# schatty/oprl

Hardware: AMD Instinct MI355X
Metric: learner gradient steps/sec, DDPG batch=256 walker-walk (higher is better)
Workload: dtype f32 (exact-fp32 MFMA)

## Files before the change

### oprl_amd/csrc/batch_rows.h

```cpp
#pragma once
#include "kernels.h"
#include "philox.h"
#include "replay_index.h"

namespace oprl {

constexpr int kMaxEnds = 2048;

__device__ __forceinline__ void load_batch(const BatchSrc& P, int row0, int B, int S, int A,
                                           float* xa, float* xb, float* rS, float* dS, int* meta,
                                           int* endsS) {
  const int tid = threadIdx.x;
  if (P.gather) {
    lds_zero(xa, 2 * kR * kX0Ld);
    const EndsLds ET = stage_ends(P.ends, P.n_eps, endsS, kMaxEnds, tid, kThreads);
    __syncthreads();
    if (tid < kR) {
      const int i = row0 + tid;
      int e = 0, t = 0;
      if (i < B) {
        const u32x4 rnd = philox4x32_10(
            u32x4{(uint32_t)P.counter, (uint32_t)(P.counter >> 32), (uint32_t)i, 0x5a17u},
            (uint32_t)P.seed, (uint32_t)(P.seed >> 32));
        const long ind = (long)bounded_u32(rnd.x, (uint32_t)P.n_transitions);
        long start = 0;
        e = find_episode(P.ends, P.n_eps, ET, ind, &start);
        t = (int)(ind - start);
      }
      meta[tid] = e;
      meta[kR + tid] = t;
    }
    __syncthreads();
    for (int idx = tid; idx < kR * (2 * S + A + 2); idx += kThreads) {
      const int W = 2 * S + A + 2;
      const int row = idx / W, c = idx - row * W;
      if (row0 + row >= B) continue;
      const long e = meta[row], t = meta[kR + row];
      const float* src = P.states + (e * (P.L + 1) + t) * S + c;
      float* dst = xa + row * kX0Ld + c;
      if (c >= S) dst = xb + row * kX0Ld + (c - S);
      if (c >= 2 * S) { src = P.actions + (e * P.L + t) * A + (c - 2 * S); dst = xa + row * kX0Ld + S + (c - 2 * S); }
      if (c == 2 * S + A) { src = P.rewards + e * P.L + t; dst = rS + row; }
      if (c == 2 * S + A + 1) { src = P.dones + e * P.L + t; dst = dS + row; }
      *dst = *src;
    }
  } else {
    constexpr int kPer = (2 * kR * kX0Ld + kThreads - 1) / kThreads;
    float v[kPer];
#pragma unroll
    for (int j = 0; j < kPer; ++j) {
      const int idx = min(tid + j * kThreads, 2 * kR * kX0Ld - 1);
      const int t = idx / (kR * kX0Ld), rem = idx - t * (kR * kX0Ld);
      const int row = rem / kX0Ld, col = rem - row * kX0Ld, gr = row0 + row;
      const bool is_s = gr < B && col < S, is_a = gr < B && t == 0 && col >= S && col < S + A;
      const float* src = P.s;
      if (is_s) src = (t == 0 ? P.s : P.s2) + (size_t)gr * S + col;
      if (is_a) src = P.a + (size_t)gr * A + (col - S);
      const float x = *src;
      v[j] = (is_s || is_a) ? x : 0.f;
    }
#pragma unroll
    for (int j = 0; j < kPer; ++j) {
      const int idx = tid + j * kThreads;
      if (idx < 2 * kR * kX0Ld) xa[idx] = v[j];
    }
    if (tid < kR) {
      const int gr = row0 + tid;
      rS[tid] = gr < B ? P.r[gr] : 0.f;
      dS[tid] = gr < B ? P.d[gr] : 0.f;
    }
  }
}

template <bool WT = false>
__device__ __forceinline__ void prefetch_rows_src(const BatchSrc& N, int S, int Ad, int B, int slice, float* smem);
__device__ __forceinline__ void prefetch_rows_body(const PrefetchJob& J, int slice, float* smem) {
  prefetch_rows_src(J.next, J.S, J.A, J.B, slice, smem);
}
template <bool WT>
__device__ __forceinline__ void prefetch_rows_src(const BatchSrc& N, int S, int Ad, int B, int slice, float* smem) {
  const int tid = threadIdx.x, row0 = slice * kR;
  float* xa = smem;
  float* xb = xa + kR * kX0Ld;
  float* rS = xb + kR * kX0Ld;
  float* dS = rS + kR;
  int* meta = reinterpret_cast<int*>(dS + 2 * kR);
  int* endsS = reinterpret_cast<int*>(rS + 96);
  load_batch(N, row0, B, S, Ad, xa, xb, rS, dS, meta, endsS);
  __syncthreads();
  if constexpr (WT) {
    store_rows_wt(xa, kX0Ld, const_cast<float*>(N.s), S, S, row0, B);
    store_rows_wt(xb, kX0Ld, const_cast<float*>(N.s2), S, S, row0, B);
    store_rows_wt(xa + S, kX0Ld, const_cast<float*>(N.a), Ad, Ad, row0, B);
    if (tid < kR && row0 + tid < B) {
      __hip_atomic_store(const_cast<float*>(N.r) + row0 + tid, rS[tid], __ATOMIC_RELAXED, __HIP_MEMORY_SCOPE_AGENT);
      __hip_atomic_store(const_cast<float*>(N.d) + row0 + tid, dS[tid], __ATOMIC_RELAXED, __HIP_MEMORY_SCOPE_AGENT);
    }
    return;
  }
  store_rows(xa, kX0Ld, const_cast<float*>(N.s), S, S, row0, B);
  store_rows(xb, kX0Ld, const_cast<float*>(N.s2), S, S, row0, B);
  for (int idx = tid; idx < kR * Ad; idx += kThreads) {
    const int row = idx / Ad, col = idx - row * Ad, gr = row0 + row;
    if (gr < B) const_cast<float*>(N.a)[(size_t)gr * Ad + col] = xa[row * kX0Ld + S + col];
  }
  if (tid < kR && row0 + tid < B) {
    const_cast<float*>(N.r)[row0 + tid] = rS[tid];
    const_cast<float*>(N.d)[row0 + tid] = dS[tid];
  }
}

__device__ __forceinline__ void prefetch_rows_direct(const PrefetchJob& J, int slice, int* lds_i, int nt) {
  const int tid = threadIdx.x, row0 = slice * kR, S = J.S, Ad = J.A, B = J.B;
  const BatchSrc& P = J.next;
  int* endsS = lds_i;
  int* meta = lds_i + kMaxEnds;
  const EndsLds ET = stage_ends(P.ends, P.n_eps, endsS, kMaxEnds, tid, nt);
  __syncthreads();
  if (tid < kR) {
    const int i = row0 + tid;
    int e = 0, t = 0;
    if (i < B) {
// ... 28 lines not shown
```

### oprl_amd/csrc/dw_tile_x2.h

```cpp
#pragma once
#include "dw_body.h"

namespace oprl {

constexpr int kDwX2TileK = 64;

__device__ __forceinline__ float wave_max(float v) {
  v = fmaxf(v, __builtin_bit_cast(float, __builtin_amdgcn_update_dpp(0, __builtin_bit_cast(int, v), 0xB1, 0xF, 0xF, true)));
  v = fmaxf(v, __builtin_bit_cast(float, __builtin_amdgcn_update_dpp(0, __builtin_bit_cast(int, v), 0x4E, 0xF, 0xF, true)));
  v = fmaxf(v, __builtin_bit_cast(float, __builtin_amdgcn_update_dpp(0, __builtin_bit_cast(int, v), 0x141, 0xF, 0xF, true)));
  v = fmaxf(v, __builtin_bit_cast(float, __builtin_amdgcn_update_dpp(0, __builtin_bit_cast(int, v), 0x140, 0xF, 0xF, true)));
  const int b = __builtin_bit_cast(int, v);
  const float r0 = __builtin_bit_cast(float, __builtin_amdgcn_readlane(b, 0)), r1 = __builtin_bit_cast(float, __builtin_amdgcn_readlane(b, 16));
  const float r2 = __builtin_bit_cast(float, __builtin_amdgcn_readlane(b, 32)), r3 = __builtin_bit_cast(float, __builtin_amdgcn_readlane(b, 48));
  return fmaxf(fmaxf(r0, r1), fmaxf(r2, r3));
}

__device__ __forceinline__ float ld_ag(const float* p) { return __hip_atomic_load(p, __ATOMIC_RELAXED, __HIP_MEMORY_SCOPE_AGENT); }
__device__ __forceinline__ void st_ag(float* p, float v) { __hip_atomic_store(p, v, __ATOMIC_RELAXED, __HIP_MEMORY_SCOPE_AGENT); }
template <class V16>
__device__ __forceinline__ void st16_wt(float* base, size_t off, const V16 v) {
  static_assert(sizeof(V16) == 16, "16-byte vector");
  st16_agent_at(base, (unsigned)off, __builtin_bit_cast(f32x4, v));
}
// ... 388 lines not shown
      unsigned long long x = 0, xb = 0;
      bool ok = false;
      for (int spin = 0; spin < (1 << 20) && !ok; ++spin) {
        x = __hip_atomic_load(src + tid, __ATOMIC_RELAXED, __HIP_MEMORY_SCOPE_SYSTEM);
        xb = tid < kDwTileN ? __hip_atomic_load(src + 1024 + tid, __ATOMIC_RELAXED, __HIP_MEMORY_SCOPE_SYSTEM) : x;
        ok = (unsigned)(x >> 32) == tag && (unsigned)(xb >> 32) == tag;
        if (!ok) __builtin_amdgcn_s_sleep(2);
      }
      *v = __uint_as_float((unsigned)x);
      *vb = __uint_as_float((unsigned)xb);
      return ok;
    };
    float gs = 0.f, gbs = 0.f;
    bool all_ok = true;
    if (X.rank == owner) {
      for (int r = 0; r < X.world; ++r) {
        float v = gsum, vb = gbw;
        if (r != X.rank) all_ok = get(slot(X.window, r), &v, &vb) && all_ok;
        gs += v;
        gbs += vb;
      }
      if (!all_ok) { gs = __builtin_nanf(""); gbs = gs; }
      for (int p = 0; p < X.world; ++p)
        if (p != X.rank) put(slot(X.peer[p], X.world), gs, gbs);
    } else {
      put(slot(X.peer[owner], X.rank), gsum, gbw);
      all_ok = get(slot(X.window, X.world), &gs, &gbs);
    }
    if (!all_ok) {
      report_expired(X.err, (KERN_DW_XCHG << 8) | SITE_DW_TILE);
      gs = __builtin_nanf(""); gbs = gs;
    }
    gsum = gs;
    gb_x = gbs;
  }
  gsum *= ad.grad_scale;
  if (!ad.do_adam) {
    if (e_ok && I.w_g != nullptr) I.w_g[eo] = gsum;
    if (b_own && I.b_g != nullptr) {
      float gb = 0.f;
#pragma unroll
      for (int q = 0; q < 32; ++q) gb += bpart[q * 16 + tid];
      I.b_g[n_base + tid] = gb * ad.grad_scale;
    }
    return;
  }
  float th_new = 0.f, tt_new = 0.f;
  if (e_ok) {
    float mm = p_m, vv = p_v, th = p_th;
    adam_elem(gsum, mm, vv, th, ad, step_size, bc2_sqrt);
    th_new = th;
    if (polyak) tt_new = polyak_elem(p_tt, th, ad);
    e_m = mm; e_v = vv;
    if (!flagged) {
      st_ag(I.w_m + eo, mm);
      st_ag(I.w_v + eo, vv);
      st_ag(I.w + eo, th);
      if (polyak) st_ag(I.w_t + eo, tt_new);
    }
    if (chained && gate == 2 && kind == 0) st_ag(ov.chain->w3buf[(ov.u + 1) & 1] + eo, th);
  }
  tileW[nl * LDT + kl] = th_new;
  tileT[nl * LDT + kl] = tt_new;
  if (b_own) {
    const int n = n_base + tid;
    float gb = 0.f;
#pragma unroll
    for (int q = 0; q < 32; ++q) gb += bpart[q * 16 + tid];
    if (xchg_on) gb = gb_x;
    gb *= ad.grad_scale;
    float mm = q_m, vv = q_v, th = q_th;
    adam_elem(gb, mm, vv, th, ad, step_size, bc2_sqrt);
    if (I.b16 != nullptr) st_ag(I.b16 + n, th);
    st_ag(I.b_m + n, mm);
    st_ag(I.b_v + n, vv);
    st_ag(I.b + n, th);
    if (b_pol) {
      const float tb = polyak_elem(q_tt, th, ad);
      st_ag(I.b_t + n, tb);
      if (I.bt16 != nullptr) st_ag(I.bt16 + n, tb);
    }
  }
  __syncthreads();

  if constexpr (!P::kX2) {
    if (I.pf != nullptr) {
      const int NSk = cdiv(I.K, 16), NSn = cdiv(I.N, 16);
      const int grp3 = tid >> 8, q = tid & 255, j = q >> 6, l = q & 63, li = l & 15, lk = l >> 4;
      if (grp3 < 2) {
        float* dst = grp3 == 0 ? I.pf : (polyak ? I.tpf : nullptr);
        if (dst != nullptr && 4 * tk + j < NSk && !(flagged && grp3 == 1))
          st16_wt(dst, (((size_t)ptile * NSk + 4 * tk + j) * 64 + l) * 4, ld4((grp3 == 0 ? tileW : tileT) + li * LDT + 16 * j + 4 * lk));
      } else if (grp3 == 2 && I.pb != nullptr) {
        const int ktile = 4 * tk + j;
        if (16 * ktile < I.K) {
          f32x4 w4;
#pragma unroll
          for (int t = 0; t < 4; ++t) w4[t] = tileW[(4 * lk + t) * LDT + 16 * j + li];
          st16_wt(I.pb, (((size_t)ktile * NSn + ptile) * 64 + l) * 4, w4);
        }
      }
    }
  }
  if (!P::kX2 && I.pf16 != nullptr && !I.x2) {
    const int NSk2 = cdiv(I.K, 32), NSn2 = cdiv(I.N, 32);
    typedef __bf16 bf16x4 __attribute__((ext_vector_type(4)));
    if (tid < 256) {
      const int which = tid >> 7, hb = (tid >> 6) & 1, l = tid & 63, li = l & 15, lk = l >> 4;
      float* dst = which == 0 ? I.pf16 : (polyak ? I.tpf16 : nullptr);
      if (dst != nullptr && 2 * tk + hb < NSk2) {
        const float* src = (which == 0 ? tileW : tileT) + li * LDT + 32 * hb;
        st16_wt(dst, (((size_t)ptile * NSk2 + 2 * tk + hb) * 64 + l) * 4, cvt_bf16x8(ld4(src + 4 * lk), ld4(src + 16 + 4 * lk)));
      }
    } else if (tid < 512 && I.pb16 != nullptr) {
      const int q = tid - 256, blk = q >> 6, l = q & 63, li = l & 15, lk = l >> 4;
      const int ktile = 4 * tk + blk;
      if (16 * ktile < I.K) {
        f32x4 w4;
#pragma unroll
        for (int t = 0; t < 4; ++t) w4[t] = tileW[(4 * lk + t) * LDT + 16 * blk + li];
        st8_wt(I.pb16 + (((size_t)ktile * NSn2 + (n_base >> 5)) * 64 + l) * 4 + 2 * ((n_base >> 4) & 1), __builtin_convertvector(w4, bf16x4));
      }
    }
  }
  if (P::kX2 && I.pf16 != nullptr) {
    const int NSk2 = cdiv(I.K, 32), NSn2 = cdiv(I.N, 32);
    typedef _Float16 f16x4 __attribute__((ext_vector_type(4)));
    if (tid < 256) {
      const int which = tid >> 7, hb = (tid >> 6) & 1, l = tid & 63, li = l & 15, lk = l >> 4;
      float* dst = which == 0 ? I.pf16 : (polyak ? I.tpf16 : nullptr);
      if (dst != nullptr && 2 * tk + hb < NSk2 && !(flagged && which == 1)) {
        const float* src = (which == 0 ? tileW : tileT) + li * LDT + 32 * hb;
        f16x8 hi, lo;
        x2_split8(ld4(src + 4 * lk) * PrecX2::kWScale, ld4(src + 16 + 4 * lk) * PrecX2::kWScale, hi, lo);
        const size_t d = ((size_t)ptile * NSk2 + 2 * tk + hb) * 512 + (size_t)l * 4;
        st16_wt(dst, d, hi);
        st16_wt(dst, d + 256, lo);
      }
    } else if (tid < 512 && I.pb16 != nullptr) {
      const int q = tid - 256, blk = q >> 6, l = q & 63, li = l & 15, lk = l >> 4;
      const int ktile = 4 * tk + blk;
      if (16 * ktile < I.K) {
        f32x4 w4;
#pragma unroll
        for (int t = 0; t < 4; ++t) w4[t] = tileW[(4 * lk + t) * LDT + 16 * blk + li];
        const f32x4 vs = w4 * PrecX2::kWScale;
        const f16x4 hi = __builtin_convertvector(vs, f16x4);
        const f32x4 r = vs - __builtin_convertvector(hi, f32x4);
        float* d = I.pb16 + ((size_t)ktile * NSn2 + (n_base >> 5)) * 512 + (size_t)l * 4 + 2 * ((n_base >> 4) & 1);
        st8_wt(d, hi);
        st8_wt(d + 256, __builtin_convertvector(r, f16x4));
      }
    }
  }
  if (flagged) {
    asm volatile("s_waitcnt vmcnt(0)" ::: "memory");
    __syncthreads();
    if (tid == 0)
      __hip_atomic_store(G.done + bx_, (unsigned long long)gtag << 32, __ATOMIC_RELAXED, __HIP_MEMORY_SCOPE_AGENT);
    if (e_ok) {
      st_ag(I.w_m + eo, e_m);
      st_ag(I.w_v + eo, e_v);
      st_ag(I.w + eo, th_new);
      if (polyak) st_ag(I.w_t + eo, tt_new);
    }
    if constexpr (!P::kX2) {
      if (I.pf != nullptr && polyak && I.tpf != nullptr && tid >= 256 && tid < 512) {
        const int NSk = cdiv(I.K, 16);
        const int q = tid & 255, j = q >> 6, l = q & 63, li = l & 15, lk = l >> 4;
        if (4 * tk + j < NSk)
          st16_wt(I.tpf, (((size_t)ptile * NSk + 4 * tk + j) * 64 + l) * 4, ld4(tileT + li * LDT + 16 * j + 4 * lk));
      }
    }
    if (P::kX2 && I.pf16 != nullptr && polyak && I.tpf16 != nullptr && tid >= 128 && tid < 256) {
      const int NSk2 = cdiv(I.K, 32);
      const int hb = (tid >> 6) & 1, l = tid & 63, li = l & 15, lk = l >> 4;
      if (2 * tk + hb < NSk2) {
        const float* src = tileT + li * LDT + 32 * hb;
        f16x8 hi, lo;
        x2_split8(ld4(src + 4 * lk) * PrecX2::kWScale, ld4(src + 16 + 4 * lk) * PrecX2::kWScale, hi, lo);
        const size_t d = ((size_t)ptile * NSk2 + 2 * tk + hb) * 512 + (size_t)l * 4;
        st16_wt(I.tpf16, d, hi);
        st16_wt(I.tpf16, d + 256, lo);
      }
    }
  }
  stamp();
  if (chained) {
    asm volatile("s_waitcnt vmcnt(0)" ::: "memory");
    __syncthreads();
    if (tid == 0)
      __hip_atomic_store((gate == 1 ? ov.chain->ct_fin : ov.chain->at_fin) + bx_, (unsigned long long)gtag << 32, __ATOMIC_RELAXED, __HIP_MEMORY_SCOPE_AGENT);
  }
  }
};

template <class KArgs = DwKArgs, class P = PrecX2>
__device__ __forceinline__ void dw_tile_x2(const KArgs& A, float* lds, int bx, int gate, const DwX2Ovr& ov = DwX2Ovr()) {
  DwX2Tile<KArgs, P> T;
  T.ov = ov;
  T.begin(A, lds, bx, gate);
  T.finish();
}

}
```

### oprl_amd/csrc/fused_ddpg.hip

```cpp
#include <cstddef>
#include <mutex>
#include <type_traits>
#include "kernels.h"
#include "philox.h"
#include "replay_index.h"
#include "batch_rows.h"
#include "slice_head.h"
#include "tp4.h"
#include "dw_body.h"
#include "dw_tile_x2.h"

namespace oprl { constexpr bool kDwTileX2 = true; constexpr bool kMergedTile64 = true; }

namespace oprl {


__device__ __forceinline__ bool cluster_on_one_xcd(const DdpgArgs& A) {
  const int xcc = __builtin_amdgcn_s_getreg((3 << 11) | 20) & 15;
  return A.xcd_local != 0 && ((int)gridDim.x & 7) == 0 && xcc == ((int)blockIdx.x & 7);
}
__global__ void k_xcc_probe(int* out) {
  if (threadIdx.x == 0) out[blockIdx.y * gridDim.x + blockIdx.x] = __builtin_amdgcn_s_getreg((3 << 11) | 20) & 15;
}

// ... 843 lines not shown
template <int WIDTH, bool LEAN, bool SAC, class P = PrecF32, bool WIDE = false>
__global__ __launch_bounds__(kThreads) void k_ddpg_phase2(const DdpgArgs A) { ddpg_phase2_body<WIDTH, LEAN, SAC, P, WIDE>(A); }

template <int WIDTH, bool LEAN, bool SAC, class P = PrecF32>
__global__ __launch_bounds__(kThreads) void k_ddpg_phase2_group(const DdpgArgs* __restrict__ batch) {
  const int S = (int)gridDim.x, R = (int)gridDim.y, n = (int)gridDim.z;
  int l = (int)blockIdx.z, slice = (int)blockIdx.x, by = (int)blockIdx.y;
  if ((n & 7) == 0) {
    const int q = (int)blockIdx.x + S * ((int)blockIdx.y + R * (int)blockIdx.z);
    const int p = q >> 3, inner = p % (S * R);
    l = (q & 7) + 8 * (p / (S * R));
    if constexpr (LEAN) {
      if (inner < 4 * S) { slice = inner >> 2; by = inner & 3; }
      else { slice = inner - 4 * S; by = 4; }
    } else {
      slice = inner % S;
      by = inner / S;
      const int G = batch[0].group_span;
      if (G > 1 && G < 8 && S % G == 0) {
        const int Sp = S / G, pr = p % (Sp * R);
        const int v = (q & 7) + 8 * (p / (Sp * R));
        l = v / G;
        slice = (v - l * G) * Sp + pr % Sp;
        by = pr / Sp;
      } else if (G >= 8) {
        l = (int)blockIdx.z; slice = (int)blockIdx.x; by = (int)blockIdx.y;
      }
    }
  }
  ddpg_phase2_body<WIDTH, LEAN, SAC, P>(batch[l], slice, by);
}


__device__ __forceinline__ void wait_flags(const unsigned long long* flags, int n, unsigned tag, unsigned* err, unsigned code) {
  const int k = (int)threadIdx.x;
  if (k < n) {
    bool ok = false;
    for (int spin = 0; spin < kTpSpin && !ok; ++spin) {
      ok = (unsigned)(__hip_atomic_load(flags + k, __ATOMIC_RELAXED, __HIP_MEMORY_SCOPE_AGENT) >> 32) == tag;
      if (!ok) __builtin_amdgcn_s_sleep(2);
    }
    if (!ok) report_expired(err, code);
  }
}

struct PassCtx {
  unsigned epoch;
  unsigned tag;
  const float* w3;
  const float* cb[3];
  long long* trace;
  const float* pb1_32 = nullptr;
};
template <class P, class KA = DwKArgs, bool PF = true, bool GE = false>
__device__ __forceinline__ int ddpg_phase2m_body(const DdpgArgs& A, const KA* D, int by_in, const PassCtx& cx) {
  static_assert((P::kX2 || GE) && kDwTileX2, "the merged phase 2: PrecX2 learners; with the unit-seed rows (k_ddpg_chain) every arithmetic");
  extern __shared__ __attribute__((aligned(16))) float smem[];
  using LY = FusedLds<256>;
  constexpr int HB = kR * kWL4;
  constexpr int NMC = 8;
  const int B = A.B, S = A.S, Ad = A.A, tid = threadIdx.x;
  const int slice = blockIdx.x, row0 = slice * kR;
  const int y = by_in < 0 ? (int)blockIdx.y : by_in;
  const int yP = NMC, yT = yP + ((PF && A.prefetch_next) ? 1 : 0);
  if (y >= yT) {
    const int tile = (y - yT) * (int)gridDim.x + slice;
    if (tile >= dw_total(*D)) return -1;
    if (A.whole) {
      wait_flags(A.w_flags, 4 * (int)gridDim.x, cx.epoch, A.err, (KERN_PHASE2 << 8) | SITE_DW_GATE);
      __syncthreads();
    }
    return tile;
  }
  float* xa = smem + LY::xa;
  if (PF && y == yP) {
    float* xb = smem + LY::xb;
    float* rS = smem + LY::misc;
    float* dS = rS + kR;
    int* meta = reinterpret_cast<int*>(dS + 2 * kR);
    int* endsS = reinterpret_cast<int*>(smem + LY::misc + 96);
    load_batch(A.next, row0, B, S, Ad, xa, xb, rS, dS, meta, endsS);
    __syncthreads();
    store_rows(xa, kX0Ld, const_cast<float*>(A.next.s), S, S, row0, B);
    store_rows(xb, kX0Ld, const_cast<float*>(A.next.s2), S, S, row0, B);
    for (int idx = tid; idx < kR * Ad; idx += kThreads) {
      const int row = idx / Ad, col = idx - row * Ad, gr = row0 + row;
      if (gr < B) const_cast<float*>(A.next.a)[(size_t)gr * Ad + col] = xa[row * kX0Ld + S + col];
    }
    if (tid < kR && row0 + tid < B) {
      const_cast<float*>(A.next.r)[row0 + tid] = rS[tid];
      const_cast<float*>(A.next.d)[row0 + tid] = dS[tid];
    }
    return -1;
  }
  float* h1 = smem + LY::h;
  float* h2 = h1 + HB;
  float* g2 = h2 + HB;
  float* Wl = g2 + HB;
  float* outS = smem + LY::out;
  float* auxS = smem + LY::aux;
  float* duS = smem + LY::aux2;
  float* scr = smem + LY::scr;
  float* w3s = smem + LY::misc + 96;
  static_assert(2 * HB >= 2 * 8 * 512, "the shard fits the two spare hidden buffers");
  static_assert(kMaxEnds >= kDuLd * 256, "W3 fits the ends table's area");
  Tp tp{y, NMC, A.xbuf + (size_t)slice * kTpStages * A.xnc * kTpBlk, cx.tag, 0,
// ... 28 lines not shown
  const float* wsrc = ((P::kBf16 && cx.pb1_32 != nullptr) ? cx.pb1_32 : A.actor.pb[1]) + (size_t)c * 2 * 16 * 256;
  f32x4 wv[2];
#pragma unroll
  for (int q = 0; q < 2; ++q) wv[q] = ld4c(wsrc + ((size_t)q * kThreads + tid) * 4);
  const int hr = tid >> 6, hc = (tid & 63) * 4;
  f32x4 hv = f32x4{0.f, 0.f, 0.f, 0.f};
  if (row0 + hr < B) hv = ld4c(A.aX[2] + (size_t)(row0 + hr) * kW4 + hc);
  f32x4 w3q = f32x4{0.f, 0.f, 0.f, 0.f};
  if ((tid >> 6) < Ad) w3q = ld4c(cx.w3 + (size_t)tid * 4);
  const int et = (tid >> 8) & 1, er = (tid >> 4) & 15, ec = tid & 15;
  float m1 = 0.f;
  if (!GE && tid < 512 && row0 + er < B) m1 = ldc(A.aX[1] + (size_t)(row0 + er) * kW4 + 32 * c + 16 * et + ec);
  f32x4 gm1 = f32x4{0.f, 0.f, 0.f, 0.f};
  if constexpr (GE) {
#pragma unroll
    for (int r = 0; r < 4; ++r)
      if (row0 + 4 * kk + r < B) gm1[r] = ldc(A.aX[1] + (size_t)(row0 + 4 * kk + r) * kW4 + 32 * c + 16 * (wave & 1) + i);
  }
  const int rs_ = tid / S, cs_ = tid - rs_ * S;
  const bool oks = tid < kR * S && row0 + rs_ < B;
  const float vs = oks ? ldc(A.aX[0] + (size_t)(row0 + rs_) * A.aldx0 + cs_) : 0.f;
  const int tid2 = tid + kThreads;
  const int rs2_ = tid2 / S, cs2_ = tid2 - rs2_ * S;
  const bool oks2 = tid2 < kR * S && row0 + rs2_ < B;
  const float vs2 = oks2 ? ldc(A.aX[0] + (size_t)(row0 + rs2_) * A.aldx0 + cs2_) : 0.f;
  const int rp_ = tid / Ad, cp_ = tid - rp_ * Ad;
  const bool okp = tid < kR * Ad && row0 + rp_ < B;
  const float vp = okp ? ldc(A.pi + (size_t)(row0 + rp_) * Ad + cp_) : 0.f;
  lds_zero(xa, kR * kX0Ld);
  lds_zero(auxS, kR * kOutLd);
  __syncthreads();
  if (tid < kR * S) xa[rs_ * kX0Ld + cs_] = vs;
  if (tid2 < kR * S) xa[rs2_ * kX0Ld + cs2_] = vs2;
  if (tid < kR * Ad) xa[rp_ * kX0Ld + S + cp_] = vp;
#pragma unroll
  for (int q = 0; q < 2; ++q) *reinterpret_cast<f32x4*>(Wl + ((size_t)q * kThreads + tid) * 4) = wv[q];
  if (tid < kDuLd * 64) *reinterpret_cast<f32x4*>(w3s + (size_t)tid * 4) = w3q;
  const unsigned mbits = (hv[0] > 0.f ? 1u : 0u) | (hv[1] > 0.f ? 2u : 0u) | (hv[2] > 0.f ? 4u : 0u) | (hv[3] > 0.f ? 8u : 0u) |
                         (m1 > 0.f ? 16u : 0u);
  stamp();
  if constexpr (GE && !P::kX2) {
    float* mS = h1;
    *reinterpret_cast<f32x4*>(mS + hr * kWL4 + hc) = f32x4{(mbits & 1u) ? 1.f : 0.f, (mbits & 2u) ? 1.f : 0.f, (mbits & 4u) ? 1.f : 0.f, (mbits & 8u) ? 1.f : 0.f};
    __syncthreads();
    const int t1 = wave & 1, j = wave >> 1;
    if (j < Ad) {
      f32x4 acc0 = f32x4{0.f, 0.f, 0.f, 0.f}, acc1 = acc0;
#pragma unroll 4
      for (int sx = 0; sx < 16; ++sx) {
        const f32x4 b4 = ld4(Wl + ((size_t)t1 * 16 + sx) * 256 + lane * 4);
        const f32x4 a4 = ld4(mS + i * kWL4 + 16 * sx + 4 * kk) * ld4(w3s + j * 256 + 16 * sx + 4 * kk);
        if (sx & 1) { mac4(a4, b4, acc1); } else { mac4(a4, b4, acc0); }
      }
#pragma unroll
      for (int r = 0; r < 4; ++r)
        if (row0 + 4 * kk + r < B)
          st_ag(A.gu + ((size_t)j * B + row0 + 4 * kk + r) * kW4 + 32 * c + 16 * t1 + i, gm1[r] > 0.f ? acc0[r] + acc1[r] : 0.f);
    }
    stamp();
  }
  if constexpr (GE && P::kX2) {
    typedef _Float16 f16x4 __attribute__((ext_vector_type(4)));
    _Float16* mH = reinterpret_cast<_Float16*>(h1);
    _Float16* wH = reinterpret_cast<_Float16*>(h1 + 2048);
    _Float16* wL = reinterpret_cast<_Float16*>(h1 + 2048 + 1024);
    float* sJ = h1 + 2048 + 2048;
    static_assert(HB >= 2048 + 2048 + 16, "masks and the output layer's planes fit one hidden buffer");
    {
      const int l = tid & 63, ws_ = l >> 3, half_ = (l >> 2) & 1, kq_ = l & 3;
      const int off = ((ws_ * 4 + kq_) * 8) + 4 * half_;
      union { f16x4 v; unsigned short b[4]; } mk;
#pragma unroll
      for (int t = 0; t < 4; ++t) mk.b[t] = ((mbits >> t) & 1u) ? 0xffffu : 0u;
      *reinterpret_cast<f16x4*>(mH + hr * 256 + off) = mk.v;
      if ((tid >> 6) < kDuLd) {
        float m = fmaxf(fmaxf(fabsf(w3q[0]), fabsf(w3q[1])), fmaxf(fabsf(w3q[2]), fabsf(w3q[3])));
        m = wave_max(m);
        const float sj = P::a_scale(m);
        f16x8 hi8, lo8;
        x2_split8(w3q * sj, f32x4{0.f, 0.f, 0.f, 0.f}, hi8, lo8);
        *reinterpret_cast<f16x4*>(wH + (tid >> 6) * 256 + off) = __builtin_shufflevector(hi8, hi8, 0, 1, 2, 3);
        *reinterpret_cast<f16x4*>(wL + (tid >> 6) * 256 + off) = __builtin_shufflevector(lo8, lo8, 0, 1, 2, 3);
        if (l == 0) sJ[tid >> 6] = sj;
      }
    }
    __syncthreads();
    const int t1 = wave & 1, j = wave >> 1;
    if (j < Ad) {
      f32x4 acc = f32x4{0.f, 0.f, 0.f, 0.f};
      typedef unsigned u32x4v __attribute__((ext_vector_type(4)));
#pragma unroll
      for (int ws = 0; ws < 8; ++ws) {
        const float* bw = Wl + ((size_t)t1 * 8 + ws) * 512 + lane * 4;
        const f16x8 bh = __builtin_bit_cast(f16x8, ld4(bw)), bl = __builtin_bit_cast(f16x8, ld4(bw + 256));
        const u32x4v mk = *reinterpret_cast<const u32x4v*>(mH + i * 256 + (ws * 4 + kk) * 8);
        const u32x4v h4 = *reinterpret_cast<const u32x4v*>(wH + j * 256 + (ws * 4 + kk) * 8);
        const u32x4v l4 = *reinterpret_cast<const u32x4v*>(wL + j * 256 + (ws * 4 + kk) * 8);
        const f16x8 ah = __builtin_bit_cast(f16x8, h4 & mk), al = __builtin_bit_cast(f16x8, l4 & mk);
        acc = __builtin_amdgcn_mfma_f32_16x16x32_f16(al, bh, acc, 0, 0, 0);
        acc = __builtin_amdgcn_mfma_f32_16x16x32_f16(ah, bl, acc, 0, 0, 0);
        acc = __builtin_amdgcn_mfma_f32_16x16x32_f16(ah, bh, acc, 0, 0, 0);
      }
      const float un = PrecX2::kOut / sJ[j];
#pragma unroll
      for (int r = 0; r < 4; ++r)
        if (row0 + 4 * kk + r < B)
          st_ag(A.gu + ((size_t)j * B + row0 + 4 * kk + r) * kW4 + 32 * c + 16 * t1 + i, gm1[r] > 0.f ? acc[r] * un : 0.f);
    }
    stamp();
  }
  if (A.whole) {
    if (tid < A.n_ct && A.debug_expire != 102) {
      bool ok = false;
      for (int spin = 0; spin < kTpSpin && !ok; ++spin) {
        ok = (unsigned)(__hip_atomic_load(A.ct_done + tid, __ATOMIC_RELAXED, __HIP_MEMORY_SCOPE_AGENT) >> 32) == cx.epoch;
        if (!ok) __builtin_amdgcn_s_sleep(1);
      }
      if (!ok) report_expired(A.err, (KERN_PHASE2 << 8) | SITE_DW_GATE);
    }
    __syncthreads();
    cbo.b0 = cx.cb[0]; cbo.b1 = cx.cb[1]; cbo.b2 = cx.cb[2];
  }
  if constexpr (GE) {
    asm volatile("s_waitcnt vmcnt(0)" ::: "memory");
    __syncthreads();
    if (tid == 0)
      __hip_atomic_store(A.gu_flags + slice * NMC + c, (unsigned long long)cx.epoch << 32, __ATOMIC_RELAXED, __HIP_MEMORY_SCOPE_AGENT);
  }
  stamp();
  float* qsum = nullptr;
  if (A.partials_a != nullptr && lead) {
    qsum = A.partials_a + slice * 4 + 1;
    if (tid == 0) { A.partials_a[slice * 4 + 0] = 0.f; A.partials_a[slice * 4 + 2] = 0.f; }
  }
  tp4_scalar_fb<typename std::conditional<GE, Coh<P>, P>::type, NMC>(A.critic, xa, h1, h2, g2, outS, scr, tp, nostore, row0, B, -A.inv_B, S, Ad, auxS, stamp, qsum, cbo);
  stamp();
  if (lead && okp) {
    const float du = auxS[rp_ * kOutLd + cp_] * (1.f - vp * vp);
    granule_put(A.du_granules + (size_t)(row0 + rp_) * kDuLd + cp_, cx.epoch, du);
    A.adY[2][(size_t)(row0 + rp_) * A.alddo + cp_] = du;
  }
  if constexpr (GE) { stamp(); return -1; }
  if constexpr (P::kX2 && !GE) {
    f32x4 gq = f32x4{0.f, 0.f, 0.f, 0.f};
    const bool row_in = row0 + hr < B;
#pragma unroll
    for (int j = 0; j < kDuLd; ++j) {
      float d = 0.f;
      if (j < Ad && row_in) {
        const float pv = xa[hr * kX0Ld + S + j];
        d = auxS[hr * kOutLd + j] * (1.f - pv * pv);
      }
      gq += ld4(w3s + j * 256 + hc) * d;
    }
#pragma unroll
    for (int t = 0; t < 4; ++t) gq[t] = ((mbits >> t) & 1u) != 0u ? gq[t] : 0.f;
    float m = fmaxf(fmaxf(fabsf(gq[0]), fabsf(gq[1])), fmaxf(fabsf(gq[2]), fabsf(gq[3])));
    m = wave_max(m);
    const float sr = P::a_scale(m);
    *reinterpret_cast<f32x4*>(h1 + hr * kWL4 + hc) = gq * sr;
// ... 58 lines not shown
}

template <class P>
__global__ __launch_bounds__(kThreads) void k_ddpg_chain(const DdpgArgs A, const DwKArgs4 Dc, const DwKArgs4 Da, const ChainArgs C_) {
  static_assert(kDwTileX2, "the chain launch runs the 16 x 64 tiles of dw_tile_x2.h");
  extern __shared__ __attribute__((aligned(16))) float smem[];
  const char* ka = (const char*)__builtin_amdgcn_kernarg_segment_ptr();
  const DwKArgs4* Dcp = (const DwKArgs4*)(ka + kWholeDcOffset);
  const DwKArgs4* Dap = (const DwKArgs4*)(ka + kWholeDaOffset);
  const ChainArgs& C = *(const ChainArgs*)(ka + kChainCOffset);
  using LY = FusedLds<256>;
  constexpr int HB = kR * kWL4;
  const int slices = (int)gridDim.x, slice = (int)blockIdx.x;
  const int R = C.rows;
  const int u = (int)blockIdx.y / R, yy = chain_row((int)blockIdx.y - u * R, C.order);
  const int B = A.B, S = A.S, Ad = A.A, tid = threadIdx.x, row0 = slice * kR;
  const unsigned ep = A.epoch + (unsigned)u;
  const unsigned tag1 = A.cluster_tag + 2u * (unsigned)u, tag2 = tag1 + 1u;
  const int tc = Dcp->tile_end[kDwFusedItems - 1], ta = Dap->tile_end[kDwFusedItems - 1];
  const int par = u & 1;
  float* xa = smem + LY::xa;
  float* xb = smem + LY::xb;
  float* h1 = smem + LY::h;
  float* h2 = h1 + HB;
  float* outS = smem + LY::out;
  float* scr = smem + LY::scr;
  float* rS = smem + LY::misc;
  float* dS = rS + kR;
  float* yS = dS + kR;
  int* meta = reinterpret_cast<int*>(yS + kR);
  int* endsS = reinterpret_cast<int*>(smem + LY::misc + 96);
  const int role = yy < 8 ? 0 : (yy < 12 ? 1 : (yy < 16 ? 2 : 3));
  const int member = yy < 8 ? yy : (yy < 16 ? (yy - 8) & 3 : 1);
  const bool lead = member == 0;
  const int spin = A.debug_expire == (int)SITE_CLUSTER ? 0 : kTpSpin;
  const bool traced = kTraceOn && A.trace != nullptr && u == C.trace_u;
  int n_stamp = 0;
  auto stamp = [&]() {
    if (traced && role < 3 && (tid & 63) == 0 && (tid == 0 || slice == 0) && lead && n_stamp < kTraceStamps) {
      const int slot = tid == 0 ? slice : 16 + (tid >> 6);
      long long* tr = A.trace + (((size_t)role * 64 + slot) * kTraceStamps + n_stamp) * 2;
      tr[0] = (long long)__builtin_readcyclecounter();
      tr[1] = (long long)wall_clock64();
    }
    ++n_stamp;
  };
  stamp();

  if (u > 0 && role == 0) chain_wait2(C.pf_done + slice, 1, nullptr, 0, nullptr, 0, ep - 1u, A.err, (KERN_PHASE1 << 8) | SITE_DW_GATE);
  if (u > 0 && role != 0) chain_wait2(C.ct_fin, tc, C.at_fin, role == 1 ? 0 : ta, C.pf_done + slice, role == 3 ? 0 : 1, ep - 1u, A.err, (KERN_PHASE1 << 8) | SITE_DW_GATE);
  if (role == 3) {
  } else if (u == 0 && C.first_gather) {
    load_batch(A.src, row0, B, S, Ad, xa, xb, rS, dS, meta, endsS);
  } else {
    const float* ps = par ? C.set1[0] : C.set0[0]; const float* pa = par ? C.set1[1] : C.set0[1];
    const float* pr = par ? C.set1[2] : C.set0[2]; const float* pd = par ? C.set1[3] : C.set0[3];
    const float* ps2 = par ? C.set1[4] : C.set0[4];
    lds_zero(xa, 2 * kR * kX0Ld);
    __syncthreads();
    load_rows_c(xa, kX0Ld, 0, ps, S, S, row0, B);
    load_rows_c(xa, kX0Ld, S, pa, Ad, Ad, row0, B);
    load_rows_c(xb, kX0Ld, 0, ps2, S, S, row0, B);
    if (tid < kR) {
      const int gr = row0 + tid;
      rS[tid] = gr < B ? ldc(pr + gr) : 0.f;
      dS[tid] = gr < B ? ldc(pd + gr) : 0.f;
    }
  }
  stamp();
  if (u > 0 && role == 0) {
    __syncthreads();
    chain_wait2(C.ct_fin, tc, C.at_fin, ta, nullptr, 0, ep - 1u, A.err, (KERN_PHASE1 << 8) | SITE_DW_GATE);
  }
  stamp();
  const Tp3Store nostore{nullptr, nullptr, nullptr, nullptr, 0};
  auto bias_of = [&](int which) {
    BiasOv bo;
    if (u > 0) { bo.b0 = C.b16[which][0]; bo.b1 = C.b16[which][1]; bo.b2 = C.b16[which][2]; }
    return bo;
  };

  if (role == 0) {
    Tp tp{member, 8, A.xbuf + (size_t)slice * kTpStages * A.xnc * kTpBlk, tag1, 0, A.err, KERN_PHASE1 << 8, spin};
    tp.local = cluster_on_one_xcd(A);
    tp4_forward<Coh<P>, 8>(A.actor_t, xb, h1, h2, outS, scr, tp, nostore, row0, B, stamp, bias_of(1));
    for (int idx = tid; idx < kR * Ad; idx += kThreads) {
      const int row = idx / Ad, col = idx - row * Ad, gr = row0 + row;
      xb[row * kX0Ld + S + col] = gr < B ? tanhf(outS[row * kOutLd + col]) : 0.f;
    }
    unsigned long long gq[4] = {0ull, 0ull, 0ull, 0ull};
    float qb = 0.f;
    int hook_n = 0;
    const unsigned long long* gq_src = C.qp + (size_t)slice * 64 + (tid & (kR - 1));
    auto hook = [&]() {
      stamp();
      if (++hook_n == 2) {
#pragma unroll
        for (int m = 0; m < 4; ++m) gq[m] = __hip_atomic_load(gq_src + m * kR, __ATOMIC_RELAXED, __HIP_MEMORY_SCOPE_AGENT);
        qb = ldc(u > 0 ? C.b16[2][2] : A.critic.b[2]);
      }
    };
    tp4_forward<Coh<P>, 8>(A.critic_t, xb, h1, h2, outS, scr, tp, nostore, row0, B, hook, bias_of(3));
    if (lead && tid < 64) {
      const int gr = row0 + tid;
      const bool row_ok = tid < kR && gr < B;
      const float qn = row_ok ? outS[tid * kOutLd] : 0.f;
      const float y = row_ok ? rS[tid] + ((1.f - dS[tid]) * A.gamma) * qn : 0.f;
      const int lim = A.debug_expire == (int)SITE_TD_TARGET ? 0 : (1 << 20);
      float q = 0.f;
      if (row_ok) {
        bool ok = lim > 0;
#pragma unroll
        for (int m = 0; m < 4; ++m) ok = ok && (unsigned)(gq[m] >> 32) == ep;
        if (A.debug_expire == 101) ok = true;
        for (int sp = 0; sp < lim && !ok; ++sp) {
#pragma unroll
          for (int m = 0; m < 4; ++m) gq[m] = __hip_atomic_load(gq_src + m * kR, __ATOMIC_RELAXED, __HIP_MEMORY_SCOPE_AGENT);
          ok = true;
#pragma unroll
          for (int m = 0; m < 4; ++m) ok = ok && (unsigned)(gq[m] >> 32) == ep;
          if (!ok) __builtin_amdgcn_s_sleep(1);
        }
        if (!ok) report_expired(A.err, (KERN_PHASE1 << 8) | SITE_TD_TARGET);
        float qs = 0.f;
#pragma unroll
        for (int m = 0; m < 4; ++m) qs += __uint_as_float((unsigned)gq[m]);
        q = ok ? qs + qb : __builtin_nanf("");
        const float seed = 2.f * (q - y) * A.inv_B;
        A.cdY[2][(size_t)gr * A.clddo] = seed;
        __hip_atomic_store(A.y_granules + gr, ((unsigned long long)ep << 32) | (unsigned long long)__float_as_uint(seed),
                           __ATOMIC_RELAXED, __HIP_MEMORY_SCOPE_AGENT);
        if (A.y_out != nullptr) A.y_out[gr] = y;
        if (A.q_out != nullptr) A.q_out[gr] = q;
      }
      if (A.partials_c != nullptr) {
        float v[3] = {row_ok ? (q - y) * (q - y) : 0.f, row_ok ? q : 0.f, row_ok ? y : 0.f};
#pragma unroll
        for (int k = 0; k < 3; ++k) {
          const float sum = row16_sum(v[k]);
          if (tid == 0) A.partials_c[(size_t)slice * 4 + k] = sum;
        }
      }
    }
    stamp();
    __syncthreads();
    int by2 = (int)blockIdx.y;
    asm volatile("" : "+s"(by2));
    const int u2 = by2 / C.rows;
    const PassCtx cx{A.epoch + (unsigned)u2, A.cluster_tag + 2u * (unsigned)u2 + 1u, C.w3buf[u2 & 1], {C.b16[2][0], C.b16[2][1], C.b16[2][2]},
                     (kTraceOn && u2 == C.trace_u) ? A.trace2 : nullptr, A.actor_pb1_f32};
    (void)ddpg_phase2m_body<P, DwKArgs4, false, true>(A, Dap, chain_row(by2 - u2 * C.rows, C.order), cx);
    return;
  }

  if (role == 1) {
    Tp tp{member, 4, A.xbuf + ((size_t)1 * slices + slice) * kTpStages * A.xnc * kTpBlk, tag1, 0, A.err, KERN_PHASE1 << 8, spin};
    tp.local = cluster_on_one_xcd(A);
    const Tp3Store st{A.cX[1], A.cX[2], A.cdY[1], A.cdY[0], A.cdY0_stride, B, true};
    if (lead) {
      __syncthreads();
      for (int idx = tid; idx < kR * (S + Ad); idx += kThreads) {
        const int row = idx / (S + Ad), col = idx - row * (S + Ad), gr = row0 + row;
        if (gr < B) __hip_atomic_store(A.cX[0] + (size_t)gr * A.cldx0 + col, xa[row * kX0Ld + col], __ATOMIC_RELAXED, __HIP_MEMORY_SCOPE_AGENT);
      }
    }
    const QPart qp{C.qp + (size_t)slice * 64, ep};
    tp4_scalar_fb<Coh<P>>(A.critic, xa, h1, h2, h1 + 2 * HB, outS, scr, tp, st, row0, B, 1.f, 0, 0, nullptr, stamp, nullptr, bias_of(2), qp);
    asm volatile("s_waitcnt vmcnt(0)" ::: "memory");
    __syncthreads();
    if (tid == 0)
      __hip_atomic_store(A.gate_flags + slice * 4 + member, (unsigned long long)ep << 32, __ATOMIC_RELAXED, __HIP_MEMORY_SCOPE_AGENT);
    stamp();
  } else if (role == 2) {
    Tp tp{member, 4, A.xbuf + ((size_t)2 * slices + slice) * kTpStages * A.xnc * kTpBlk, tag1, 0, A.err, KERN_PHASE1 << 8, spin};
    tp.local = cluster_on_one_xcd(A);
    const Tp3Store st{A.aX[1], A.aX[2], nullptr, nullptr, 0, 0, true};
    tp4_forward<Coh<P>>(A.actor, xa, h1, h2, outS, scr, tp, st, row0, B, stamp, bias_of(0));
    if (lead) {
      for (int idx = tid; idx < kR * Ad; idx += kThreads) {
        const int row = idx / Ad, col = idx - row * Ad, gr = row0 + row;
        if (gr < B) st_ag(A.pi + (size_t)gr * Ad + col, tanhf(outS[row * kOutLd + col]));
      }
      store_rows_wt(xa, kX0Ld, A.aX[0], A.aldx0, S, row0, B);
      if (u == 0 && slice == 0)
        for (int idx = tid * 4; idx < Ad * kW4; idx += kThreads * 4)
          st16_wt(C.w3buf[0], idx, ld4(A.w3_src + idx));
    }
    stamp();
    asm volatile("s_waitcnt vmcnt(0)" ::: "memory");
    __syncthreads();
    if (tid == 0)
      __hip_atomic_store(A.w_flags + slice * 4 + member, (unsigned long long)ep << 32, __ATOMIC_RELAXED, __HIP_MEMORY_SCOPE_AGENT);
  }
  __syncthreads();
  int by2 = (int)blockIdx.y, bx2 = (int)blockIdx.x, nx2 = (int)gridDim.x;
  asm volatile("" : "+s"(by2), "+s"(bx2), "+s"(nx2));
  const int u2 = by2 / C.rows, y2 = chain_row(by2 - u2 * C.rows, C.order);
  const int wg2 = y2 < 16 ? ((y2 >= 12) ? 4 * nx2 : 0) + bx2 * 4 + ((y2 - 8) & 3) : 8 * nx2 + (y2 - 16) * nx2 + bx2;
  const int n_bc = 8 * nx2;
  const unsigned ep2 = A.epoch + (unsigned)u2;

  {
    const int p = n_bc + (C.rows - 16) * nx2 - 1 - wg2;
    if (p >= 0 && p < nx2 && (u2 + 1 < C.n_upd || C.pf_last)) {
      const int par2 = u2 & 1;
      BatchSrc nx = A.next;
      nx.s = par2 ? C.set0[0] : C.set1[0]; nx.a = par2 ? C.set0[1] : C.set1[1]; nx.r = par2 ? C.set0[2] : C.set1[2];
      nx.d = par2 ? C.set0[3] : C.set1[3]; nx.s2 = par2 ? C.set0[4] : C.set1[4];
      nx.counter = A.next.counter + (unsigned long long)u2;
      prefetch_rows_src<true>(nx, A.S, A.A, A.B, p, smem);
      asm volatile("s_waitcnt vmcnt(0)" ::: "memory");
      __syncthreads();
      if (threadIdx.x == 0)
        __hip_atomic_store(C.pf_done + p, (unsigned long long)ep2 << 32, __ATOMIC_RELAXED, __HIP_MEMORY_SCOPE_AGENT);
    }
  }
  {
    const int tile = wg2 < Dcp->tile_end[kDwFusedItems - 1] ? wg2 : -1;
    if (tile >= 0) {
      DwX2Ovr ov;
      ov.chain = &C; ov.u = u2;
      dw_tile_x2<DwKArgs4, P>(*Dcp, smem, tile, 1, ov);
    }
  }
  {
    int by3 = (int)blockIdx.y, bx3 = (int)blockIdx.x, nx3 = (int)gridDim.x;
    asm volatile("" : "+s"(by3), "+s"(bx3), "+s"(nx3));
    const int u3 = by3 / C.rows, y3 = chain_row(by3 - u3 * C.rows, C.order);
    const int wg3 = y3 < 16 ? ((y3 >= 12) ? 4 * nx3 : 0) + bx3 * 4 + ((y3 - 8) & 3) : 8 * nx3 + (y3 - 16) * nx3 + bx3;
    const int tile = wg3 < Dap->tile_end[kDwFusedItems - 1] ? wg3 : -1;
// ... 284 lines not shown
```

Before: 34800.

## Coalesce weight/optimizer writebacks and defer batch staging into forward pipelines

Adam state and weight writebacks in the dW tile are staged through LDS and written back as 16-byte write-through stores instead of per-element scalar stores. The gu gradient stores are transposed through per-wave scratch so each lane emits one 16-byte store. For roles 1 and 2, batch row staging is moved from the kernel prologue into a callback run inside the forward pipelines, using coherent loads, and the critic input copy is folded into that staging. The aim is fewer, wider global transactions and hiding batch loads behind pipeline work. The cost is extra LDS traffic and new wave-barrier synchronisation, and the callback API changes in tp4_forward and tp4_scalar_fb are not visible here.

```diff
diff --git a/oprl_amd/csrc/batch_rows.h b/oprl_amd/csrc/batch_rows.h
--- a/oprl_amd/csrc/batch_rows.h
+++ b/oprl_amd/csrc/batch_rows.h
@@ -68,6 +68,36 @@
       const int gr = row0 + tid;
       rS[tid] = gr < B ? P.r[gr] : 0.f;
       dS[tid] = gr < B ? P.d[gr] : 0.f;
+    }
+  }
+}
+
+__device__ __forceinline__ void load_xa_coherent(const float* s, const float* a, int row0, int B, int S, int A, float* xa,
+                                                 float* out, int ldo) {
+  const int tid = threadIdx.x;
+  constexpr int kPer = (kR * kX0Ld + kThreads - 1) / kThreads;
+  float v[kPer];
+  bool in[kPer];
+#pragma unroll
+  for (int j = 0; j < kPer; ++j) {
+    const int idx = min(tid + j * kThreads, kR * kX0Ld - 1);
+    const int row = idx / kX0Ld, col = idx - row * kX0Ld, gr = row0 + row;
+    const bool is_s = gr < B && col < S, is_a = gr < B && col >= S && col < S + A;
+    const float* src = s;
+    if (is_s) src = s + (size_t)gr * S + col;
+    if (is_a) src = a + (size_t)gr * A + (col - S);
+    const float x = ldc(src);
+    in[j] = is_s || is_a;
+    v[j] = in[j] ? x : 0.f;
+  }
+#pragma unroll
+  for (int j = 0; j < kPer; ++j) {
+    const int idx = tid + j * kThreads;
+    if (idx < kR * kX0Ld) {
+      xa[idx] = v[j];
+      const int row = idx / kX0Ld, col = idx - row * kX0Ld;
+      if (out != nullptr && in[j])
+        __hip_atomic_store(out + (size_t)(row0 + row) * ldo + col, v[j], __ATOMIC_RELAXED, __HIP_MEMORY_SCOPE_AGENT);
     }
   }
 }
diff --git a/oprl_amd/csrc/dw_tile_x2.h b/oprl_amd/csrc/dw_tile_x2.h
--- a/oprl_amd/csrc/dw_tile_x2.h
+++ b/oprl_amd/csrc/dw_tile_x2.h
@@ -464,16 +464,12 @@
     th_new = th;
     if (polyak) tt_new = polyak_elem(p_tt, th, ad);
     e_m = mm; e_v = vv;
-    if (!flagged) {
-      st_ag(I.w_m + eo, mm);
-      st_ag(I.w_v + eo, vv);
-      st_ag(I.w + eo, th);
-      if (polyak) st_ag(I.w_t + eo, tt_new);
-    }
     if (chained && gate == 2 && kind == 0) st_ag(ov.chain->w3buf[(ov.u + 1) & 1] + eo, th);
   }
   tileW[nl * LDT + kl] = th_new;
   tileT[nl * LDT + kl] = tt_new;
+  part[nl * LDT + kl] = e_m;
+  part[(16 + nl) * LDT + kl] = e_v;
   if (b_own) {
     const int n = n_base + tid;
     float gb = 0.f;
@@ -570,12 +566,44 @@
     __syncthreads();
     if (tid == 0)
       __hip_atomic_store(G.done + bx_, (unsigned long long)gtag << 32, __ATOMIC_RELAXED, __HIP_MEMORY_SCOPE_AGENT);
-    if (e_ok) {
-      st_ag(I.w_m + eo, e_m);
-      st_ag(I.w_v + eo, e_v);
-      st_ag(I.w + eo, th_new);
-      if (polyak) st_ag(I.w_t + eo, tt_new);
-    }
+  }
+  const bool wide = (tiles_k == 1 || (I.K & 3) == 0) &&
+                    ((((size_t)I.w_m | (size_t)I.w_v | (size_t)I.w | (polyak ? (size_t)I.w_t : (size_t)0)) & 15) == 0);
+  if (wide) {
+    const int arr = tid >> 8, q = tid & 255;
+    float* dst = arr == 0 ? I.w_m : (arr == 1 ? I.w_v : (arr == 2 ? I.w : (polyak ? I.w_t : nullptr)));
+    const float* src = arr == 0 ? part : (arr == 1 ? part + 16 * LDT : (arr == 2 ? tileW : tileT));
+    if (dst != nullptr && tiles_k == 1) {
+      const int rows = min(kDwTileN, I.N - n_base), span = rows * I.K, f0 = 4 * q;
+      if (f0 < span) {
+        int r = f0 / I.K, c = f0 - r * I.K;
+        f32x4 v;
+#pragma unroll
+        for (int t = 0; t < 4; ++t) {
+          v[t] = src[r * LDT + c];
+          if (++c == I.K) { c = 0; ++r; }
+        }
+        const size_t o = (size_t)n_base * I.K + f0;
+        if (f0 + 3 < span) {
+          st16_wt(dst, o, v);
+        } else {
+#pragma unroll
+          for (int t = 0; t < 4; ++t)
+            if (f0 + t < span) st_ag(dst + o + t, v[t]);
+        }
+      }
+    } else if (dst != nullptr) {
+      const int r = q >> 4, c = (q & 15) * 4;
+      if (n_base + r < I.N && k_base + c < I.K)
+        st16_wt(dst, (size_t)(n_base + r) * I.K + k_base + c, ld4(src + r * LDT + c));
+    }
+  } else if (e_ok) {
+    st_ag(I.w_m + eo, e_m);
+    st_ag(I.w_v + eo, e_v);
+    st_ag(I.w + eo, th_new);
+    if (polyak) st_ag(I.w_t + eo, tt_new);
+  }
+  if (flagged) {
     if constexpr (!P::kX2) {
       if (I.pf != nullptr && polyak && I.tpf != nullptr && tid >= 256 && tid < 512) {
         const int NSk = cdiv(I.K, 16);
diff --git a/oprl_amd/csrc/fused_ddpg.hip b/oprl_amd/csrc/fused_ddpg.hip
--- a/oprl_amd/csrc/fused_ddpg.hip
+++ b/oprl_amd/csrc/fused_ddpg.hip
@@ -919,6 +919,16 @@
   long long* trace;
   const float* pb1_32 = nullptr;
 };
+__device__ __forceinline__ void gu_store16(float* dst, float* wscr, const f32x4 v, size_t off, int rows) {
+  const int lane = threadIdx.x & 63, i = lane & 15, kk = lane >> 4;
+#pragma unroll
+  for (int r = 0; r < 4; ++r) wscr[(4 * kk + r) * 16 + i] = v[r];
+  __builtin_amdgcn_fence(__ATOMIC_RELEASE, "wavefront");
+  __builtin_amdgcn_wave_barrier();
+  __builtin_amdgcn_fence(__ATOMIC_ACQUIRE, "wavefront");
+  const int row = lane >> 2, cq = (lane & 3) * 4;
+  if (row < rows) st16_wt(dst, off + (size_t)row * kW4 + cq, ld4(wscr + row * 16 + cq));
+}
 template <class P, class KA = DwKArgs, bool PF = true, bool GE = false>
 __device__ __forceinline__ int ddpg_phase2m_body(const DdpgArgs& A, const KA* D, int by_in, const PassCtx& cx) {
   static_assert((P::kX2 || GE) && kDwTileX2, "the merged phase 2: PrecX2 learners; with the unit-seed rows (k_ddpg_chain) every arithmetic");
@@ -1053,10 +1063,10 @@
         const f32x4 a4 = ld4(mS + i * kWL4 + 16 * sx + 4 * kk) * ld4(w3s + j * 256 + 16 * sx + 4 * kk);
         if (sx & 1) { mac4(a4, b4, acc1); } else { mac4(a4, b4, acc0); }
       }
-#pragma unroll
-      for (int r = 0; r < 4; ++r)
-        if (row0 + 4 * kk + r < B)
-          st_ag(A.gu + ((size_t)j * B + row0 + 4 * kk + r) * kW4 + 32 * c + 16 * t1 + i, gm1[r] > 0.f ? acc0[r] + acc1[r] : 0.f);
+      f32x4 gv;
+#pragma unroll
+      for (int r = 0; r < 4; ++r) gv[r] = gm1[r] > 0.f ? acc0[r] + acc1[r] : 0.f;
+      gu_store16(A.gu, scr + wave * 256, gv, ((size_t)j * B + row0) * kW4 + 32 * c + 16 * t1, B - row0);
     }
     stamp();
   }
@@ -1103,10 +1113,10 @@
         acc = __builtin_amdgcn_mfma_f32_16x16x32_f16(ah, bh, acc, 0, 0, 0);
       }
       const float un = PrecX2::kOut / sJ[j];
-#pragma unroll
-      for (int r = 0; r < 4; ++r)
-        if (row0 + 4 * kk + r < B)
-          st_ag(A.gu + ((size_t)j * B + row0 + 4 * kk + r) * kW4 + 32 * c + 16 * t1 + i, gm1[r] > 0.f ? acc[r] * un : 0.f);
+      f32x4 gv;
+#pragma unroll
+      for (int r = 0; r < 4; ++r) gv[r] = gm1[r] > 0.f ? acc[r] * un : 0.f;
+      gu_store16(A.gu, scr + wave * 256, gv, ((size_t)j * B + row0) * kW4 + 32 * c + 16 * t1, B - row0);
     }
     stamp();
   }
@@ -1271,6 +1281,7 @@
   if (role == 3) {
   } else if (u == 0 && C.first_gather) {
     load_batch(A.src, row0, B, S, Ad, xa, xb, rS, dS, meta, endsS);
+  } else if (role != 0) {
   } else {
     const float* ps = par ? C.set1[0] : C.set0[0]; const float* pa = par ? C.set1[1] : C.set0[1];
     const float* pr = par ? C.set1[2] : C.set0[2]; const float* pd = par ? C.set1[3] : C.set0[3];
@@ -1297,6 +1308,17 @@
     BiasOv bo;
     if (u > 0) { bo.b0 = C.b16[which][0]; bo.b1 = C.b16[which][1]; bo.b2 = C.b16[which][2]; }
     return bo;
+  };
+  auto stage_xa = [&]() {
+    if (!(u == 0 && C.first_gather)) {
+      int by = (int)blockIdx.y, bx = (int)blockIdx.x;
+      asm volatile("" : "+s"(by), "+s"(bx));
+      const ChainArgs& Cc = *(const ChainArgs*)((const char*)__builtin_amdgcn_kernarg_segment_ptr() + kChainCOffset);
+      const DdpgArgs& Aa = *(const DdpgArgs*)__builtin_amdgcn_kernarg_segment_ptr();
+      const int uu = by / Cc.rows, y = chain_row(by - uu * Cc.rows, Cc.order);
+      const float* const* set = (uu & 1) ? Cc.set1 : Cc.set0;
+      load_xa_coherent(set[0], set[1], bx * kR, Aa.B, Aa.S, Aa.A, smem + LY::xa, y == 8 ? Aa.cX[0] : nullptr, Aa.cldx0);
+    }
   };
 
   if (role == 0) {
@@ -1376,7 +1398,7 @@
     Tp tp{member, 4, A.xbuf + ((size_t)1 * slices + slice) * kTpStages * A.xnc * kTpBlk, tag1, 0, A.err, KERN_PHASE1 << 8, spin};
     tp.local = cluster_on_one_xcd(A);
     const Tp3Store st{A.cX[1], A.cX[2], A.cdY[1], A.cdY[0], A.cdY0_stride, B, true};
-    if (lead) {
+    if (lead && u == 0 && C.first_gather) {
       __syncthreads();
       for (int idx = tid; idx < kR * (S + Ad); idx += kThreads) {
         const int row = idx / (S + Ad), col = idx - row * (S + Ad), gr = row0 + row;
@@ -1384,7 +1406,7 @@
       }
     }
     const QPart qp{C.qp + (size_t)slice * 64, ep};
-    tp4_scalar_fb<Coh<P>>(A.critic, xa, h1, h2, h1 + 2 * HB, outS, scr, tp, st, row0, B, 1.f, 0, 0, nullptr, stamp, nullptr, bias_of(2), qp);
+    tp4_scalar_fb<Coh<P>>(A.critic, xa, h1, h2, h1 + 2 * HB, outS, scr, tp, st, row0, B, 1.f, 0, 0, nullptr, stamp, nullptr, bias_of(2), qp, stage_xa);
     asm volatile("s_waitcnt vmcnt(0)" ::: "memory");
     __syncthreads();
     if (tid == 0)
@@ -1394,7 +1416,7 @@
     Tp tp{member, 4, A.xbuf + ((size_t)2 * slices + slice) * kTpStages * A.xnc * kTpBlk, tag1, 0, A.err, KERN_PHASE1 << 8, spin};
     tp.local = cluster_on_one_xcd(A);
     const Tp3Store st{A.aX[1], A.aX[2], nullptr, nullptr, 0, 0, true};
-    tp4_forward<Coh<P>>(A.actor, xa, h1, h2, outS, scr, tp, st, row0, B, stamp, bias_of(0));
+    tp4_forward<Coh<P>>(A.actor, xa, h1, h2, outS, scr, tp, st, row0, B, stamp, bias_of(0), stage_xa);
     if (lead) {
       for (int idx = tid; idx < kR * Ad; idx += kThreads) {
         const int row = idx / Ad, col = idx - row * Ad, gr = row0 + row;
```

After: 34970, median of 6. About the same (+0.5%).
